# Parskatt/RoMa

Measured on AMD Instinct MI355X. Metric: image-pairs/sec, roma_outdoor 560->864, batch=8 per GPU, higher is better.
Workload: dtype bf16; 1 GPU; roma_outdoor match() 560->864, symmetric, upsample_preds, 8 pairs/GPU/step, seeded synthetic weights + N(0,1) images; precision policy of the reference's bf16 timing script: bfloat16 DINOv2 + float16 autocast for VGG / decoder / refiners (ROMA_MIXED), f32 accumulate; precision_policy=mixed, global_batch=8, streams_per_gpu=2, parallelism=single GPU, outputs_finite=True

## Files before the change

### include/roma_hip.h

```cpp
#ifndef ROMA_HIP_H
#define ROMA_HIP_H
#include <stdint.h>
#ifdef __cplusplus
extern "C" {
#endif

typedef struct roma_model* roma_handle_t;

enum { ROMA_F32 = 0, ROMA_BF16 = 1, ROMA_F16 = 2,
       ROMA_MIXED = 3 };
int roma_h16_format(void);
enum { ROMA_ERR_ARG = -1, ROMA_ERR_HIP = -2, ROMA_ERR_STATE = -3 };

typedef struct {
  int coarse_h, coarse_w;
  int upsample_h, upsample_w;
  int symmetric;
  int upsample_preds;
  int attenuate_cert;
  int precision;
  int max_batch;
  int device;
} roma_config_t;

// ... 52 lines not shown
int roma_debug_inject(roma_handle_t h, const char* name, const void* src_host, long nbytes);
long roma_debug_trace(roma_handle_t h, int slot, unsigned long long* sums_host, long max_entries, char* names_host,
                      long names_bytes);
int roma_destroy(roma_handle_t h);
int roma_tuning(const char* key, int value);
long roma_tuning_describe(char* buf, long nbytes);
long roma_debug_gemm_trace(unsigned int* dst_host, long nbytes);
int roma_profile_enable(int on);
long roma_profile_report(char* buf, long nbytes);


int roma_op_local_corr(const void* feature0, const void* feature1, const float* warp, void* out, int B, int H, int W,
                       int C, int K, int nearest, int dt_in, int dt_out, void* stream);
int roma_op_local_corr_window(const void* feature0, const void* feature1, const float* warp, void* out, int B, int H,
                              int W, int C, int radius, float scale, long ldo, int dt_in, int dt_out, void* stream);

int roma_op_gemm(const void* A, long lda, const void* W, long ldw, void* C, long ldc, int M, int N, int K, int batch,
                 long sA, long sW, long sC, const float* bias, const float* scale, const float* res, long ldr,
                 int act, float alpha, int dt_in, int dt_out, void* stream);
int roma_op_conv3x3(const void* in, const void* w, const float* bias, void* out, int B, int H, int W, int Cin, int Cout,
                    int relu, int dt, void* stream);
int roma_op_conv3x3_slab(const void* in, const void* w, const float* bias, void* out, int B, int H, int W, int Cin, int Cout,
                         int relu, int dt, void* stream);
int roma_op_attention(const void* q, const void* k, const void* vt, void* out, int B, int heads, int N, int npad, int hd,
                      int dt_in, int dt_out, void* stream);
int roma_op_qkv_scatter_gemm(const void* A, const void* W, const float* bias, void* q, void* k, void* vt, int B, int N,
                             int npad, int heads, int hd, int K, int dt_in, int dt_out, void* stream);
int roma_op_layernorm(const float* x, const float* w, const float* b, void* out, long M, int D, float eps, int dt_out,
                      void* stream);
int roma_op_layernorm_dt(const void* x, int dt_in, const float* w, const float* b, void* out, long M, int D, float eps,
// ... 107 lines not shown
```

### roma_amd/_lib.py

```python
from __future__ import annotations

import ctypes as C
import os

_HERE = os.path.dirname(os.path.abspath(__file__))
_HERE = os.environ.get("ROMA_LIB_DIR", _HERE)
LIB_PATH = os.path.join(_HERE, "libroma_hip.so")
LIB_PATHS = {"bf16": LIB_PATH, "f16": os.path.join(_HERE, "libroma_hip_f16.so")}

ROMA_F32, ROMA_BF16, ROMA_F16, ROMA_MIXED = 0, 1, 2, 3
H16_CODE = {"bf16": ROMA_BF16, "f16": ROMA_F16}


class RomaConfig(C.Structure):
    _fields_ = [("coarse_h", C.c_int), ("coarse_w", C.c_int), ("upsample_h", C.c_int), ("upsample_w", C.c_int),
                ("symmetric", C.c_int), ("upsample_preds", C.c_int), ("attenuate_cert", C.c_int),
                ("precision", C.c_int), ("max_batch", C.c_int), ("device", C.c_int)]


class RomaForwardArgs(C.Structure):
    _fields_ = [("upsample", C.c_int), ("symmetric", C.c_int), ("scale_factor", C.c_double),
                ("seed_flow", C.c_void_p), ("seed_cert", C.c_void_p), ("seed_h", C.c_int), ("seed_w", C.c_int),
                ("flow", C.c_void_p * 5), ("cert", C.c_void_p * 5), ("feat", C.c_void_p * 5)]

# ... 14 lines not shown
    "roma_match": (_i, [_vp, _i, _vp, _vp, _vp, _vp, _vp, _vp, _vp]),
    "roma_forward": (_i, [_vp, _i, _vp, _vp, C.POINTER(RomaForwardArgs), _vp]),
    "roma_debug_fetch": (_l, [_vp, C.c_char_p, _vp, _l]),
    "roma_debug_trace": (_l, [_vp, _i, _vp, _l, C.c_char_p, _l]),
    "roma_debug_inject": (_i, [_vp, C.c_char_p, _vp, _l]),
    "roma_destroy": (_i, [_vp]),
    "roma_tuning": (_i, [C.c_char_p, _i]),
    "roma_tuning_describe": (_l, [C.c_char_p, _l]),
    "roma_debug_gemm_trace": (_l, [_vp, _l]),
    "roma_vit_forward": (_i, [_vp, _vp]),
    "roma_op_convert_from_bf16": (_i, [_vp, _vp, _l, _vp]),
    "roma_profile_enable": (_i, [_i]),
    "roma_profile_report": (_l, [C.c_char_p, _l]),
    "roma_op_local_corr": (_i, [_vp, _vp, _vp, _vp, _i, _i, _i, _i, _i, _i, _i, _i, _vp]),
    "roma_op_local_corr_window": (_i, [_vp, _vp, _vp, _vp, _i, _i, _i, _i, _i, _f, _l, _i, _i, _vp]),
    "roma_op_gemm": (_i, [_vp, _l, _vp, _l, _vp, _l, _i, _i, _i, _i, _l, _l, _l, _vp, _vp, _vp, _l, _i, _f, _i, _i, _vp]),
    "roma_op_conv3x3": (_i, [_vp, _vp, _vp, _vp, _i, _i, _i, _i, _i, _i, _i, _vp]),
    "roma_op_conv3x3_slab": (_i, [_vp, _vp, _vp, _vp, _i, _i, _i, _i, _i, _i, _i, _vp]),
    "roma_op_attention": (_i, [_vp, _vp, _vp, _vp, _i, _i, _i, _i, _i, _i, _i, _vp]),
    "roma_op_qkv_scatter_gemm": (_i, [_vp, _vp, _vp, _vp, _vp, _vp, _i, _i, _i, _i, _i, _i, _i, _i, _vp]),
    "roma_op_layernorm": (_i, [_vp, _vp, _vp, _vp, _l, _i, _f, _i, _vp]),
    "roma_op_layernorm_dt": (_i, [_vp, _i, _vp, _vp, _vp, _l, _i, _f, _i, _vp]),
    "roma_op_gemm_res_bf16": (_i, [_vp, _l, _vp, _l, _vp, _l, _i, _i, _i, _vp, _vp, _vp, _l, _vp]),
    "roma_op_cholesky_solve_t": (_i, [_vp, _vp, _vp, _vp, _vp, _i, _i, _i, _vp]),
    "roma_op_gp": (_i, [_vp, _vp, _vp, _vp, _vp, _i, _i, _i, _i, _vp]),
    "roma_op_cls_to_flow": (_i, [_vp, _l, _vp, _vp, _l, _vp]),
    "roma_op_resize_bilinear": (_i, [_vp, _vp, _i, _i, _i, _i, _i, _i, _vp]),
    "roma_op_refiner_input": (_i, [_vp, _l, _vp, _vp, _l, _vp, _vp, _i, _i, _i, _i, _i, _i, _i, _i, _f, _i, _vp]),
    "roma_op_dwconv5x5": (_i, [_vp, _vp, _vp, _vp, _i, _i, _i, _i, _i, _vp]),
    "roma_op_refiner_block": (_i, [_vp, _vp, _vp, _vp, _vp, _vp, _i, _i, _i, _i, _i, _vp]),
# ... 86 lines not shown
```

### roma_amd/csrc/api.hip

```cpp
#include <algorithm>
#include <mutex>
#include <map>
#include <vector>
#include <dlfcn.h>
#include <string.h>

#include "../../include/roma_hip.h"
#include "attention.h"
#include "conv64.h"
#include "conv_patch.h"
#include "elementwise.h"
#include "gemm.h"
#include "local_corr.h"
#include "pool_proj.h"
#include "model.h"
#include "refiner_block.h"
#include "kde.h"
#include "keypoints.h"
#include "tiny.h"
#include "tuning.h"
#include "vit.h"
#include "sampling.h"
#include "sample_batched.h"
#include "essential.h"
// ... 286 lines not shown
  a.nearest = nearest ? 1 : 0;
  a.f0 = feature0; a.f1 = feature1; a.warp = warp; a.out = out; a.B = B; a.H = H; a.W = W; a.C = C; a.K = K;
  a.ld0 = C; a.ld1 = C; a.ldo = K; a.nimg = B; a.f1_shift = 0; a.scale = 1.f; a.in_dt = DT(dt_in); a.out_dt = DT(dt_out);
  return local_corr_general_launch(a, S(stream));
}

int roma_op_local_corr_window(const void* feature0, const void* feature1, const float* warp, void* out, int B, int H,
                              int W, int C, int radius, float scale, long ldo, int dt_in, int dt_out, void* stream) {
  LocalCorrArgs a;
  a.f0 = feature0; a.f1 = feature1; a.warp = warp; a.out = out; a.B = B; a.H = H; a.W = W; a.C = C; a.radius = radius;
  a.ld0 = C; a.ld1 = C; a.ldo = ldo; a.nimg = B; a.f1_shift = 0; a.scale = scale; a.in_dt = DT(dt_in); a.out_dt = DT(dt_out);
  ROMA_REQUIRE(ldo >= (2 * radius + 1) * (2 * radius + 1), "local_corr_window: ldo < K");
  return local_corr_window_launch(a, S(stream));
}

int roma_op_gemm(const void* A, long lda, const void* W, long ldw, void* C, long ldc, int M, int N, int K, int batch,
                 long sA, long sW, long sC, const float* bias, const float* scale, const float* res, long ldr, int act,
                 float alpha, int dt_in, int dt_out, void* stream) {
  GemmArgs g;
  g.A = A; g.lda = lda; g.W = W; g.ldw = ldw; g.C = C; g.ldc = ldc; g.M = M; g.N = N; g.K = K; g.batch = batch;
  g.sA = sA; g.sW = sW; g.sC = sC; g.bias = bias; g.scale = scale; g.res = res; g.ldr = ldr; g.sR = sC; g.act = act;
  g.alpha = alpha; g.in_dt = DT(dt_in); g.out_dt = DT(dt_out);
  return gemm_launch(g, S(stream));
}

int roma_op_conv3x3(const void* in, const void* w, const float* bias, void* out, int B, int H, int W, int Cin, int Cout,
                    int relu, int dt, void* stream) {
  GemmArgs g;
  g.A = in; g.W = w; g.ldw = 9 * Cin; g.C = out; g.ldc = Cout; g.M = B * H * W; g.N = Cout; g.K = 9 * Cin;
  g.in_dt = DT(dt); g.out_dt = DT(dt); g.bias = bias; g.act = relu ? ACT_RELU : ACT_NONE;
// ... 306 lines not shown
```

### roma_amd/csrc/chol_col.hip

```cpp
#include "chol_diag.h"
#include "elementwise.h"
#include "tuning.h"

namespace roma {

namespace {

struct CFrag { f32x4 v[8]; };

__device__ __forceinline__ void cc_load(CFrag& f, const float* p) {
#pragma unroll
  for (int q = 0; q < 8; ++q) f.v[q] = *reinterpret_cast<const f32x4*>(p + 4 * q);
}
__device__ __forceinline__ f32x16 cc_mfma(const CFrag& a, const CFrag& b, f32x16 acc) {
#pragma unroll
  for (int q = 0; q < 8; ++q)
#pragma unroll
    for (int u = 0; u < 4; ++u) acc = __builtin_amdgcn_mfma_f32_32x32x2f32(a.v[q][u], b.v[q][u], acc, 0, 0, 0);
  return acc;
}
__device__ __forceinline__ f32x16 cc_tile_product(const float* pa, const float* pb, int k) {
  f32x16 acc;
#pragma unroll
  for (int r = 0; r < 16; ++r) acc[r] = 0.f;
  CFrag a0, b0, a1, b1;
  if (k > 0) {
    cc_load(a0, pa);
    cc_load(b0, pb);
  }
  for (int t = 0; t < k; t += 2) {
    if (t + 1 < k) {
      cc_load(a1, pa + 64 * (t + 1));
      cc_load(b1, pb + 64 * (t + 1));
    }
    acc = cc_mfma(a0, b0, acc);
    if (t + 1 < k) {
      if (t + 2 < k) {
        cc_load(a0, pa + 64 * (t + 2));
        cc_load(b0, pb + 64 * (t + 2));
      }
      acc = cc_mfma(a1, b1, acc);
    }
  }
  return acc;
}

constexpr int CC_POLLS = 2000;

}

__global__ __launch_bounds__(256, 2) void chol_col_kernel(float* __restrict__ A, long ld, long strideA, float* __restrict__ LTm,
                                                          long strideLT, int n, float* __restrict__ Linv,
                                                          float* __restrict__ LinvT, int k, int nblk, unsigned epoch,
                                                          int use_leader) {
  constexpr int S = CHOL_S;
  __shared__ __attribute__((aligned(16))) float L[64 * S];
  __shared__ __attribute__((aligned(16))) float LT[64 * S];
  __shared__ __attribute__((aligned(16))) float XT[64 * S];
  __shared__ __attribute__((aligned(16))) float Pb[64 * S];
  __shared__ int progress;
  __shared__ int leader_ok;
  const int tid = threadIdx.x;
  const int wave = __builtin_amdgcn_readfirstlane(tid >> 6);
  const int lane = tid & 63, l31 = lane & 31, kk = lane >> 5;
  const int img = blockIdx.y;
  const bool split = use_leader && k > 0;
  const bool leader = split && blockIdx.x == 0;
  const int rb = split ? (int)blockIdx.x - 1 : (int)blockIdx.x;
  float* Ai = A + (long)img * strideA;
  const long S0 = 64l * k, R0 = 64l * (k + 1) + 64l * rb;
  unsigned* flag = reinterpret_cast<unsigned*>(LTm + (long)img * strideLT + n);
  const unsigned want = (epoch << 8) | (unsigned)(k + 1);
  float* Li = Linv + ((long)img * nblk + k) * 4096;
  float* LiT = LinvT + ((long)img * nblk + k) * 4096;
  if (tid == 0) {
    progress = -1;
    leader_ok = 0;
  }
  const int ti = wave >> 1, tj = wave & 1;

  if (!leader) {
    const float* pa = Ai + (R0 + 32 * ti + l31) * ld + 32 * kk;
    const float* pb = Ai + (S0 + 32 * tj + l31) * ld + 32 * kk;
    const f32x16 acc = cc_tile_product(pa, pb, k);
#pragma unroll
    for (int r = 0; r < 16; ++r) {
      const int row = 32 * ti + (r & 3) + 8 * (r >> 2) + 4 * kk, col = 32 * tj + l31;
      Pb[row * S + col] = Ai[(R0 + row) * ld + S0 + col] - acc[r];
    }
  }
  bool have_inverse = false;
  if (split && !leader) {
    if (tid == 0) {
      int ok = 0;
      for (int it = 0; it < CC_POLLS; ++it) {
        if (__hip_atomic_load(flag, __ATOMIC_RELAXED, __HIP_MEMORY_SCOPE_AGENT) == want) {
          ok = 1;
          break;
        }
// ... 2 lines not shown
      if (ok) __builtin_amdgcn_fence(__ATOMIC_ACQUIRE, "agent");
      leader_ok = ok;
    }
    __syncthreads();
    have_inverse = leader_ok != 0;
    if (have_inverse) {
      for (int idx = tid; idx < 64 * 16; idx += 256) {
        const int row = idx >> 4, c4 = (idx & 15) * 4;
        *reinterpret_cast<f32x4*>(&XT[row * S + c4]) = *reinterpret_cast<const f32x4*>(LiT + row * 64 + c4);
      }
    }
  }
  if (!have_inverse) {
    const float* pa = Ai + (S0 + 32 * ti + l31) * ld + 32 * kk;
    const float* pb = Ai + (S0 + 32 * tj + l31) * ld + 32 * kk;
    const f32x16 acc = cc_tile_product(pa, pb, k);
#pragma unroll
    for (int r = 0; r < 16; ++r) {
      const int row = 32 * ti + (r & 3) + 8 * (r >> 2) + 4 * kk, col = 32 * tj + l31;
      L[row * S + col] = Ai[(S0 + row) * ld + S0 + col] - acc[r];
    }
    __syncthreads();
    if (wave == 0) chol_diag_factor_wave(L, LT, &progress, lane);
    else if (wave == 1) chol_diag_inverse_wave(L, XT, &progress, lane);
  }
  __syncthreads();

  if (leader || (!split && rb == 0)) {
    chol_diag_writeback(L, XT, nullptr, ld, Li, LiT, tid, 256);
    float* ltd = LTm + (long)img * strideLT + S0 * (long)n + S0;
    for (int idx = tid; idx < 64 * 16; idx += 256) {
// ... 42 lines not shown
__global__ __launch_bounds__(256) void chol_col_restore_kernel(float* __restrict__ A, long ld, long strideA,
                                                               const float* __restrict__ LTm, long strideLT, int n) {
  __shared__ float tile[64 * 65];
  const int k = blockIdx.x, img = blockIdx.y, tid = threadIdx.x;
  const float* src = LTm + (long)img * strideLT + (64l * k) * n + 64l * k;
  float* dst = A + (long)img * strideA + (64l * k) * ld + 64l * k;
  for (int idx = tid; idx < 64 * 64; idx += 256) {
    const int r = idx >> 6, c = idx & 63;
    tile[r * 65 + c] = c >= r ? src[(long)r * n + c] : 0.f;
  }
  __syncthreads();
  for (int idx = tid; idx < 64 * 64; idx += 256) dst[(long)(idx >> 6) * ld + (idx & 63)] = tile[(idx & 63) * 65 + (idx >> 6)];
}

int chol_col_launch(float* A, long ld, long strideA, float* LT, long strideLT, int n, int d, float* Linv, float* LinvT, int k,
                    int nblk, int batch, unsigned epoch, hipStream_t s) {
  ROMA_REQUIRE(n % 64 == 0 && d % 64 == 0 && d >= 64 && ld % 4 == 0 && LT, "chol_col: n, d multiples of 64, d >= 64, ld of 4, LT");
  const int nrb = (n + d) / 64 - (k + 1);
  ROMA_REQUIRE(nrb >= 1 && k < nblk, "chol_col: no row block below the column");
  const int use_leader = tuning(SW_GP_COL_LEADER);
  const int gx = nrb + ((use_leader && k > 0) ? 1 : 0);
  hipLaunchKernelGGL(chol_col_kernel, dim3((unsigned)gx, (unsigned)batch), dim3(256), 0, s, A, ld, strideA, LT, strideLT, n, Linv,
                     LinvT, k, nblk, epoch & 0xffffffu, use_leader);
  ROMA_LAUNCH_CHECK();
  return 0;
}

int chol_col_restore_launch(float* A, long ld, long strideA, const float* LT, long strideLT, int n, int batch, hipStream_t s) {
  hipLaunchKernelGGL(chol_col_restore_kernel, dim3((unsigned)(n / 64), (unsigned)batch), dim3(256), 0, s, A, ld, strideA, LT,
                     strideLT, n);
  ROMA_LAUNCH_CHECK();
  return 0;
}

}
```

### roma_amd/csrc/elementwise.h

```cpp
#pragma once
#include "common.h"

namespace roma {

int layernorm_launch(const float* x, const float* w, const float* b, void* out, long M, int D, float eps,
                     int dt_out, hipStream_t s);
int layernorm_launch_dt(const void* x, int dt_in, const float* w, const float* b, void* out, long M, int D, float eps,
                        int dt_out, hipStream_t s);

int conv3x3_c3_launch(const float* img, const float* w, const float* bias, void* out, int B, int H, int W,
                      int dt_out, hipStream_t s);

int im2col3x3_c3_launch(const float* img, void* out, int B, int H, int W, int dt_out, hipStream_t s);

int maxpool2x2_launch(const void* in, void* out, int B, int H, int W, int C, int dt, hipStream_t s);

int im2col_patch14_launch(const float* img, void* out, int B, int H, int W, int Kpad, int dt_out, hipStream_t s);

int assemble_tokens_launch(const float* patch, const float* cls, const float* pos, float* tokens, int B, int T,
                           int D, hipStream_t s);

int copy2d_launch(const void* in, long ldi, int dt_in, void* out, long ldo, int dt_out, long rows, int cols,
                  hipStream_t s);

int convert_from_bf16_launch(const void* in, void* out, long n, hipStream_t s);

int rownorm_launch(const void* in, long ld, int dt, float* norms, long M, int C, hipStream_t s);

int gp_basis_launch(const float* w, const float* b, float* Ft, int Dg, int h, int wdt, int npad, hipStream_t s, int copies = 1,
                    long stride = 0);

int transpose_launch(const float* in, float* out, int n, long ld, int batch, hipStream_t s, long stride_in = 0, long stride_out = 0);

int chol_diag_launch(float* A, long ld, long strideA, float* Linv, float* LinvT, int k, int nblk, int batch,
                     hipStream_t s);

int chol_col_launch(float* A, long ld, long strideA, float* LT, long strideLT, int n, int d, float* Linv, float* LinvT, int k,
                    int nblk, int batch, unsigned epoch, hipStream_t s);
int chol_col_restore_launch(float* A, long ld, long strideA, const float* LT, long strideLT, int n, int batch, hipStream_t s);

int pad_identity_launch(float* A, long ld, long strideA, int n, int npad, int batch, hipStream_t s);

int cls_to_flow_launch(const float* logits, long ld, float* flow, float* cert, long M, hipStream_t s);

struct RefinerInputArgs {
  const void* feat = nullptr;
  long ldf = 0;
  const float* flow = nullptr;
  void* d = nullptr;
  long ldd = 0;
  const float* emb_w = nullptr;
  const float* emb_b = nullptr;
  int B = 0, H = 0, W = 0, C = 0, E = 0, Kcorr = 0, nimg = 0, shift = 0;
// ... 32 lines not shown
```

### roma_amd/csrc/local_corr.h

```cpp
#pragma once
#include "common.h"

namespace roma {

struct LocalCorrArgs {
  const void* f0 = nullptr;
  const void* f1 = nullptr;
  const float* warp = nullptr;
  void* out = nullptr;
  int B = 0, H = 0, W = 0, C = 0;
  int radius = 0;
  int K = 0;
  long ld0 = 0, ld1 = 0, ldo = 0;
  int nimg = 0, f1_shift = 0;
  float scale = 1.f;
  int in_dt = 0, out_dt = 0;
  int nearest = 0;
  int* ws = nullptr;
  long ws_bytes = 0;
  int force_gather = 0;
  int pxmax = 0;
  int bin_ts = 0, bin_nx = 0, bin_ny = 0, ws_bins = 0, ws_qlist = 0;
};

long local_corr_ws_ints(int B, int H, int W, int radius);

int local_corr_window_launch(const LocalCorrArgs& a, hipStream_t stream);
int local_corr_general_launch(const LocalCorrArgs& a, hipStream_t stream);

}
```

### roma_amd/csrc/local_corr.hip

```cpp
#include "local_corr.h"
#include "tuning.h"
#include <stdio.h>
#include <stdlib.h>
#include <algorithm>
#include "gemm.h"

namespace roma {

template <typename T> struct LcIO;
template <> struct LcIO<float> {
  static constexpr int CE = 4;
  __device__ static inline void ld(const float* p, float* v) {
    f32x4 x = *reinterpret_cast<const f32x4*>(p);
    v[0] = x[0]; v[1] = x[1]; v[2] = x[2]; v[3] = x[3];
  }
};
template <> struct LcIO<bf16_t> {
  static constexpr int CE = 8;
  __device__ static inline void ld(const bf16_t* p, float* v) {
    uint4 u = *reinterpret_cast<const uint4*>(p);
    v[0] = h16_lo(u.x); v[1] = h16_hi(u.x);
    v[2] = h16_lo(u.y); v[3] = h16_hi(u.y);
    v[4] = h16_lo(u.z); v[5] = h16_hi(u.z);
    v[6] = h16_lo(u.w); v[7] = h16_hi(u.w);
// ... 445 lines not shown
    const long bh = max(min(yhi + R + 1, a.H - 1) - max(ylo - R, 0) + 1, 0);
    coherent = bw * bh <= a.pxmax && !a.force_gather;
  }
  const unsigned long long mc = __ballot(valid && coherent), mg = __ballot(valid && !coherent);
  int basec = 0, baseg = 0;
  if (lane == 0) {
    if (mc) basec = atomicAdd(a.ws + 1, __popcll(mc));
    if (mg) baseg = atomicAdd(a.ws + 0, __popcll(mg));
  }
  basec = __shfl(basec, 0);
  baseg = __shfl(baseg, 0);
  const unsigned long long below = (1ull << lane) - 1ull;
  if (valid) {
    if (coherent) a.ws[4 + tiles + basec + __popcll(mc & below)] = tile;
    else a.ws[4 + baseg + __popcll(mg & below)] = tile;
  }
}

template <int R> __device__ __forceinline__ int lc_bin_of(const LocalCorrArgs& a, long pix, int b) {
  constexpr int P = 2 * R + 2;
  int x0, y0;
  float fx, fy;
  unnormalize_floor(a.warp[pix * 2 + 0], a.W, x0, fx);
  unnormalize_floor(a.warp[pix * 2 + 1], a.H, y0, fy);
  const int ox = min(max(x0 - R, -P), a.W), oy = min(max(y0 - R, -P), a.H);
  return (b * a.bin_ny + (oy + P) / a.bin_ts) * a.bin_nx + (ox + P) / a.bin_ts;
}

template <int R, bool SCATTER>
__global__ __launch_bounds__(64) void local_corr_bin_kernel(const LocalCorrArgs a) {
  const int li = blockIdx.x;
  const int nlist = a.ws[0];
  const int tile = a.ws[4 + li];
  if (li >= nlist) return;
  const int lane = threadIdx.x;
  const int tiles_x = (a.W + LC_TQ - 1) / LC_TQ, tiles_y = (a.H + LC_TQ - 1) / LC_TQ;
  const int tpi = tiles_x * tiles_y;
  const int b = tile / tpi;
  const int trem = tile - b * tpi;
  const int ty = trem / tiles_x, tx = trem - ty * tiles_x;
  const int gy = ty * LC_TQ + (lane >> 3), gx = tx * LC_TQ + (lane & 7);
  if (gy >= a.H || gx >= a.W) return;
  const long pix = (long)b * a.H * a.W + (long)gy * a.W + gx;
  const int bin = lc_bin_of<R>(a, pix, b);
  const int nbins = a.B * a.bin_nx * a.bin_ny;
  int* cnt = a.ws + a.ws_bins;
  if constexpr (!SCATTER) {
    atomicAdd(cnt + bin, 1);
  } else {
    const int slot = atomicAdd(cnt + 2 * nbins + bin, 1);
    a.ws[a.ws_qlist + (long)cnt[nbins + bin] * 64 + slot] = (int)pix;
  }
}

__global__ __launch_bounds__(1024) void local_corr_bin_scan_kernel(const LocalCorrArgs a) {
  __shared__ int part[1024];
  const int nbins = a.B * a.bin_nx * a.bin_ny;
  int* cnt = a.ws + a.ws_bins;
  const int tid = threadIdx.x;
  const int per = (nbins + 1023) / 1024;
  const int i0 = tid * per, i1 = min(i0 + per, nbins);
  int sum = 0;
  for (int i = i0; i < i1; ++i) sum += (cnt[i] + 63) >> 6;
  part[tid] = sum;
  __syncthreads();
  for (int off = 1; off < 1024; off <<= 1) {
    const int v = tid >= off ? part[tid - off] : 0;
    __syncthreads();
    part[tid] += v;
    __syncthreads();
  }
  int run = part[tid] - sum;
  for (int i = i0; i < i1; ++i) {
    cnt[nbins + i] = run;
    run += (cnt[i] + 63) >> 6;
  }
  if (tid == 1023) a.ws[2] = part[1023];
}

template <int R, typename T, typename TOUT, int NW>
__global__ __launch_bounds__(64 * NW) void local_corr_list_kernel(const LocalCorrArgs a) {
  extern __shared__ __attribute__((aligned(16))) float f0s[];
  constexpr int RPT = 64 / NW;
  const int li = blockIdx.x / RPT, rnd = blockIdx.x % RPT;
  const int nlist = a.ws[0];
  const int tile = a.ws[4 + li];
  if (li >= nlist) return;
  const int lane = threadIdx.x & 63, wave = threadIdx.x >> 6;
  const int tiles_x = (a.W + LC_TQ - 1) / LC_TQ, tiles_y = (a.H + LC_TQ - 1) / LC_TQ;
  const int tpi = tiles_x * tiles_y;
// ... 66 lines not shown
  ROMA_REQUIRE(a.nimg > 0, "local_corr: nimg must be positive");
  return 0;
}

static int lc_bin_ts(int radius) {
  const int P = 2 * radius + 2, pxmax = radius <= 3 ? 320 : 704;
  int ts = 1;
  while ((ts + P) * (ts + P) <= pxmax) ++ts;
  return ts;
}
long local_corr_ws_ints(int B, int H, int W, int radius) {
  if (radius != 2 && radius != 3 && radius != 7) return 0;
  const long tiles = (long)B * ((H + LC_TQ - 1) / LC_TQ) * ((W + LC_TQ - 1) / LC_TQ);
  const int ts = lc_bin_ts(radius), P = 2 * radius + 2;
  const long nbins = (long)B * ((W + P) / ts + 1) * ((H + P) / ts + 1);
  return 4 + 2 * tiles + 3 * nbins + 64 * (tiles + nbins);
}

template <int R, typename T, typename TOUT, bool MFMA>
static int launch_tiled(const LocalCorrArgs& a0, hipStream_t stream) {
  LocalCorrArgs a = a0;
  const int tiles = a.B * ((a.H + LC_TQ - 1) / LC_TQ) * ((a.W + LC_TQ - 1) / LC_TQ);
  constexpr int P = 2 * R + 2;
  a.bin_ts = lc_bin_ts(R);
  a.bin_nx = (a.W + P) / a.bin_ts + 1;
  a.bin_ny = (a.H + P) / a.bin_ts + 1;
  const long nbins = (long)a.B * a.bin_nx * a.bin_ny;
  a.ws_bins = 4 + 2 * tiles;
  a.ws_qlist = a.ws_bins + 3 * (int)nbins;
  const bool binned = tuning(SW_LC_BIN) != 0 && (long)a.B * a.H * a.W < (1l << 31) &&
                      (a.bin_ts + P - 1) * (a.bin_ts + P - 1) <= LcGeom<R, MFMA>::PXMAX;
  const size_t need = (size_t)local_corr_ws_ints(a.B, a.H, a.W, R) * sizeof(int);
  bool own_ws = false;
  if (!a.ws) {
    ROMA_CHECK_HIP(hipMallocAsync(reinterpret_cast<void**>(&a.ws), need, stream));
    own_ws = true;
  } else {
    ROMA_REQUIRE((size_t)a.ws_bytes >= need, "local_corr(window): work-list scratch too small");
  }
  a.force_gather = tuning_override(SW_LC_MODE) == 1 ? 1 : 0;
  ROMA_CHECK_HIP(hipMemsetAsync(a.ws, 0, 4 * sizeof(int), stream));
  const size_t lds_tile = (size_t)LcGeom<R, MFMA>::STAGE + 5 * 64 * 4 + 32;
  a.pxmax = LcGeom<R, MFMA>::PXMAX;
  static bool attr_set[64] = {false};
  int dev = 0;
  ROMA_CHECK_HIP(hipGetDevice(&dev));
  if (dev < 0 || dev >= 64 || !attr_set[dev]) {
    ROMA_CHECK_HIP(hipFuncSetAttribute(reinterpret_cast<const void*>(&local_corr_tile_kernel<R, T, TOUT, MFMA>),
                                       hipFuncAttributeMaxDynamicSharedMemorySize, (int)lds_tile));
    if (dev >= 0 && dev < 64) attr_set[dev] = true;
  }
  hipLaunchKernelGGL((local_corr_classify_kernel<R>), dim3((unsigned)((tiles + 63) / 64)), dim3(64), 0, stream, a);
  ROMA_LAUNCH_CHECK();
  hipLaunchKernelGGL((local_corr_tile_kernel<R, T, TOUT, MFMA>), dim3((unsigned)tiles), dim3(LcGeom<R, MFMA>::NTHR), lds_tile, stream, a);
  ROMA_LAUNCH_CHECK();
  if (binned) {
    ROMA_CHECK_HIP(hipMemsetAsync(a.ws + a.ws_bins, 0, (size_t)3 * nbins * sizeof(int), stream));
    ROMA_CHECK_HIP(hipMemsetAsync(a.ws + a.ws_qlist, 0xff, (size_t)64 * (tiles + nbins) * sizeof(int), stream));
    hipLaunchKernelGGL((local_corr_bin_kernel<R, false>), dim3((unsigned)tiles), dim3(64), 0, stream, a);
    ROMA_LAUNCH_CHECK();
    hipLaunchKernelGGL(local_corr_bin_scan_kernel, dim3(1), dim3(1024), 0, stream, a);
    ROMA_LAUNCH_CHECK();
    hipLaunchKernelGGL((local_corr_bin_kernel<R, true>), dim3((unsigned)tiles), dim3(64), 0, stream, a);
    ROMA_LAUNCH_CHECK();
    static bool attr_set_l[64] = {false};
    if (dev < 0 || dev >= 64 || !attr_set_l[dev]) {
      ROMA_CHECK_HIP(hipFuncSetAttribute(reinterpret_cast<const void*>(&local_corr_tile_kernel<R, T, TOUT, MFMA, true>),
                                         hipFuncAttributeMaxDynamicSharedMemorySize, (int)lds_tile));
      if (dev >= 0 && dev < 64) attr_set_l[dev] = true;
    }
    const long max_items = (long)tiles + nbins;
    hipLaunchKernelGGL((local_corr_tile_kernel<R, T, TOUT, MFMA, true>), dim3((unsigned)std::min<long>(max_items, 8192)), dim3(LcGeom<R, MFMA>::NTHR),
                       lds_tile, stream, a);
    ROMA_LAUNCH_CHECK();
  } else {
    hipLaunchKernelGGL((local_corr_list_kernel<R, T, TOUT, 4>), dim3((unsigned)tiles * 16u), dim3(256), (size_t)4 * a.C * sizeof(float),
                       stream, a);
    ROMA_LAUNCH_CHECK();
  }
// ... 70 lines not shown
```

### roma_amd/csrc/model.hip

```cpp
#include "model.h"

#include <dlfcn.h>
#include <math.h>
#include <stdlib.h>
#include <string.h>

#include <algorithm>
#include <atomic>
#include <set>

#include "attention.h"
#include "conv64.h"
#include "pool_proj.h"
#include "elementwise.h"
#include "gemm.h"
#include "local_corr.h"
#include "refiner_block.h"
#include "vit.h"

namespace roma {

std::mutex g_peer_mutex;
extern void* g_peer_lib;
extern int g_mixed_handles;
// ... 620 lines not shown
  return rc;
}

int cholesky_solve_t(float* A, float* Rt, float* LT, float* Linv, float* LinvT, int n, int d, int batch, hipStream_t st,
                     long strideA, long strideR) {
  ROMA_REQUIRE(n % 64 == 0 && n > 0 && d % 4 == 0, "cholesky_solve: n must be a multiple of 64, d of 4");
  const int nblk = n / 64;
  const long sA = strideA > 0 ? strideA : (long)n * n, sR = strideR > 0 ? strideR : (long)d * n, sL = (long)nblk * 4096;
  const long sLT = (long)n * n;
  const bool aug_env = tuning(SW_GP_AUG) != 0;
  const bool aug = aug_env && Rt == A + (long)n * n && (batch == 1 || (sA == sR && sA >= (long)(n + d) * n));
  const int extra = aug ? d : 0;
  const bool col = aug && tuning(SW_GP_COL) != 0 && d >= 64 && d % 64 == 0;
  static std::atomic<unsigned> solve_epoch{0};
  const unsigned epoch = col ? ++solve_epoch : 0u;
  for (int k = 0; k < nblk && col; ++k)
    if (int rc = chol_col_launch(A, n, sA, LT, sLT, n, d, Linv, LinvT, k, nblk, batch, epoch, st)) return rc;
  if (col)
    if (int rc = chol_col_restore_launch(A, n, sA, LT, sLT, n, batch, st)) return rc;
  for (int k = 0; k < nblk && !col; ++k) {
    if (int rc = chol_diag_launch(A, n, sA, Linv, LinvT, k, nblk, batch, st)) return rc;
    const int mrem = n - (k + 1) * 64;
    if (mrem + extra <= 0) break;
    GemmArgs g;
    g.A = A + (long)(k + 1) * 64 * n + k * 64; g.lda = n; g.sA = sA;
    g.W = Linv + (long)k * 4096; g.ldw = 64; g.sW = sL;
    g.C = const_cast<float*>(static_cast<const float*>(g.A)); g.ldc = n; g.sC = sA;
    g.M = mrem + extra; g.N = 64; g.K = 64; g.batch = batch;
    if (int rc = gemm_launch(g, st)) return rc;
    if (mrem <= 0) break;
    GemmArgs t;
    t.A = g.A; t.lda = n; t.sA = sA;
// ... 582 lines not shown
```

### roma_amd/csrc/tuning.hip

```cpp
#include "tuning.h"

#include <stdlib.h>
#include <string.h>

#include "../../include/roma_hip.h"

namespace roma {
void set_error(const std::string& msg);
namespace {

struct Row {
  Switch id;
  const char* key;
  const char* env;
  long def;
  int floor;
  bool tools_env;
  const char* doc;
};

constexpr Row ROWS[] = {
    {SW_GEMM8P, "gemm8p", "ROMA_GEMM8P", 1, 0, false, "large bf16 GEMMs on the 8-phase 256 x 256 kernel (1) or on the one-barrier-per-slab kernel (0)"},
    {SW_GEMM_DBG, "gemm_dbg", "ROMA_GEMM_DBG", 0, 0, false, "experiment bits of the GEMM kernels (1 skip output stores, 2 skip the K loop, 2048 no streaming stores, ...)"},
    {SW_GEMM8P_WALK, "gemm8p_walk", nullptr, -1, 1, false, "gemm8p: tile rows per group of the persistent walk (1 = row major); unset = 8 from 24 tile columns on, else 1"},
    {SW_GEMM8P_SCHED, "gemm8p_sched", "ROMA_GEMM8P_SCHED", 1, 0, false, "gemm8p K-loop schedule: 1 k-half phases, 0 quadrant phases (tools builds only)"},
    {SW_GEMM8P_MAXWG, "gemm8p_maxwg", nullptr, -1, 8, false, "gemm8p, measurement only: cap the persistent grid at n workgroups (a multiple of 8); unset = one per CU"},
    {SW_WS1X1, "ws1x1", "ROMA_WS1X1", 1, 0, false, "N = K = 576 refiner 1x1 on the weight-stationary kernel (1) or on the 256 x 192 tile kernel (0)"},
    {SW_LC_MODE, "lc_mode", "ROMA_LC_MODE", 0, 0, false, "local correlation: 0 tiled form + gather work list, 1 every tile on the gather list (key only), 2 per-pixel kernel"},
    {SW_LC_BIN, "lc_bin", "ROMA_LC_BIN", 1, 0, false, "local correlation: queries of incoherent tiles sorted by target bin (1) or gathered per query (0)"},
    {SW_CONV64, "conv64", "ROMA_CONV64", 7, 0, false, "weight-stationary VGG front end, bit mask: 1 the Cin = 64 kernels, 2 the Cin = 128 kernel, 4 the fused first layer"},
    {SW_CONV_PATCH, "conv_patch", "ROMA_CONV_PATCH", 1, 0, false, "patch-resident 3x3 kernel for slab-major VGG layers (1) or gemm8p (0); environment 0 also packs tap-major weights"},
    {SW_ATTN_XCD, "attn_xcd", "ROMA_ATTN_XCD", 1, 0, false, "attention work items in per-XCD bands of (batch, head) (1) or in plain order (0)"},
    {SW_ATTN_EXP2, "attn_exp2", nullptr, -1, 0, false, "tools only: force the 2^x softmax of the 16-bit attention kernel on / off; unset = as the caller says"},
    {SW_RB24W, "rb24w", "ROMA_RB24W", 1, 0, false, "C = 24 fused refiner block: wave-private kernel (1) or two-barrier workgroup kernel (0); consulted in tools builds only"},
    {SW_RB144_1B, "rb144_1b", "ROMA_RB144_1B", 1, 0, true, "C = 144 fused refiner block: one barrier per row (1) or two (0, tools builds only)"},
    {SW_RB_WIDE, "rb_wide", "ROMA_RB_WIDE", 0, 0, false, "C = 576 refiner block as one fused kernel (1; key 2 / 3 = with the scalar / packed stencil) or dwconv5x5 + 1x1 GEMM (0)"},
    {SW_DW_RING, "dw_ring", "ROMA_DW_RING", 1, 0, false, "depthwise 5x5: 0 register-prefetch kernel, 1 ring kernel for the large launches, 2 ring kernel for every shape it takes"},
    {SW_GP_COL, "gp_col", "ROMA_GP_COL", 1, 0, false, "GP Cholesky left-looking, one launch per block column (1) or the right-looking launch chain (0)"},
    {SW_POOL_PROJ, "pool_proj", "ROMA_POOL_PROJ", 1, 0, false, "max-pool + proj head of strides 1 / 2 in one pass (1) or as separate kernels (0)"},
    {SW_GP_COL_LEADER, "gp_col_leader", "ROMA_GP_COL_LEADER", 1, 0, false, "block-column Cholesky: one leader workgroup factorises the diagonal block (1) or every workgroup its own copy (0)"},
    {SW_GEMM8P_MINM, nullptr, "ROMA_GEMM8P_MINM", 2048, 0, false, "gemm8p: smallest M it takes for the wide (N >= 2048) dense launches"},
    {SW_GEMM_NT, nullptr, "ROMA_GEMM_NT", 1, 0, false, "non-temporal output stores in the 16-bit GEMM row writer"},
    {SW_GEMM_F32_FILL, nullptr, "ROMA_GEMM_F32_FILL", 1, 0, false, "exact-f32 GEMMs below 192 tiles of 256 x 256 run on 128 x 128 tiles"},
    {SW_GEMM_SMALLM, nullptr, "ROMA_GEMM_SMALLM", 1, 0, false, "GEMMs below 320 tiles of 128 x 128 run on 128 x 64 tiles"},
    {SW_CONV64_SY, nullptr, "ROMA_CONV64_SY", 0, 0, false, "conv64 strip height in rows; 0 = the split of H with the fewest rounds"},
    {SW_CONV_KORDER, nullptr, "ROMA_CONV_KORDER", 1, 0, false, "VGG layers with Cout >= 256 pack slab-major weight rows (read when a handle is created)"},
    {SW_RB_SY, nullptr, "ROMA_RB_SY", 0, 0, false, "fused refiner block strip height in rows; 0 = the split of H with the fewest rounds"},
    {SW_RB_DBG, nullptr, "ROMA_RB_DBG", 0, 0, true, "ablation bits of the two-barrier refiner block kernel"},
    {SW_RB_WIDE_PK, nullptr, "ROMA_RB_WIDE_PK", 1, 0, false, "rb_wide: packed (1) or scalar (0) stencil"},
    {SW_RBW_DBG, nullptr, "ROMA_RBW_DBG", 0, 0, true, "ablation bits of the rb_wide kernel (they produce wrong outputs by design)"},
    {SW_DWR_MAXSY, nullptr, "ROMA_DWR_MAXSY", 1 << 20, 0, false, "depthwise ring kernel: cap of the strip height in rows (at least 6)"},
    {SW_DW_RING_MINELEMS, nullptr, "ROMA_DW_RING_MINELEMS", 64l << 20, 0, false, "dw_ring = 1: smallest launch, in elements, that goes to the ring kernel"},
    {SW_RI_VEC, nullptr, "ROMA_RI_VEC", 1, 0, false, "refiner_input on the 16-byte vector kernel where alignment allows"},
    {SW_OUT_ROW, nullptr, "ROMA_OUT_ROW", 1, 0, false, "refiner_out: row kernel for C = 24 in 16-bit storage"},
    {SW_OUT_LPR, nullptr, "ROMA_OUT_LPR", 1, 0, false, "refiner_out, 16-bit: lanes per row chosen to fill the 16-byte pieces best"},
// ... 86 lines not shown
```

Baseline: 108.7 image-pairs/s.

## Sort local-corr queries with LDS counters and add Cholesky diagonal lookahead

The incoherent-tile binning in local correlation now runs as a banded sort kernel that counts and places queries with LDS atomics. This replaces the two workspace memsets and the per-tile device-atomic bin kernels, and a new entry point lets callers pass their own workspace. Separately, the block-column Cholesky kernel gets an extra workgroup that forms the next diagonal block's product one launch ahead and parks it, so the leader only adds the last k-slice. Both add workspace and grid complexity and change the order of floating-point accumulation.

```diff
diff --git a/include/roma_hip.h b/include/roma_hip.h
--- a/include/roma_hip.h
+++ b/include/roma_hip.h
@@ -90,6 +90,10 @@
                        int C, int K, int nearest, int dt_in, int dt_out, void* stream);
 int roma_op_local_corr_window(const void* feature0, const void* feature1, const float* warp, void* out, int B, int H,
                               int W, int C, int radius, float scale, long ldo, int dt_in, int dt_out, void* stream);
+long roma_op_local_corr_window_workspace(int B, int H, int W, int radius);
+int roma_op_local_corr_window_ws(const void* feature0, const void* feature1, const float* warp, void* out, int B, int H,
+                                 int W, int C, int radius, float scale, long ldo, int dt_in, int dt_out, void* ws,
+                                 long ws_bytes, void* stream);
 
 int roma_op_gemm(const void* A, long lda, const void* W, long ldw, void* C, long ldc, int M, int N, int K, int batch,
                  long sA, long sW, long sC, const float* bias, const float* scale, const float* res, long ldr,
diff --git a/roma_amd/_lib.py b/roma_amd/_lib.py
--- a/roma_amd/_lib.py
+++ b/roma_amd/_lib.py
@@ -52,6 +52,8 @@
     "roma_profile_report": (_l, [C.c_char_p, _l]),
     "roma_op_local_corr": (_i, [_vp, _vp, _vp, _vp, _i, _i, _i, _i, _i, _i, _i, _i, _vp]),
     "roma_op_local_corr_window": (_i, [_vp, _vp, _vp, _vp, _i, _i, _i, _i, _i, _f, _l, _i, _i, _vp]),
+    "roma_op_local_corr_window_workspace": (_l, [_i, _i, _i, _i]),
+    "roma_op_local_corr_window_ws": (_i, [_vp, _vp, _vp, _vp, _i, _i, _i, _i, _i, _f, _l, _i, _i, _vp, _l, _vp]),
     "roma_op_gemm": (_i, [_vp, _l, _vp, _l, _vp, _l, _i, _i, _i, _i, _l, _l, _l, _vp, _vp, _vp, _l, _i, _f, _i, _i, _vp]),
     "roma_op_conv3x3": (_i, [_vp, _vp, _vp, _vp, _i, _i, _i, _i, _i, _i, _i, _vp]),
     "roma_op_conv3x3_slab": (_i, [_vp, _vp, _vp, _vp, _i, _i, _i, _i, _i, _i, _i, _vp]),
diff --git a/roma_amd/csrc/api.hip b/roma_amd/csrc/api.hip
--- a/roma_amd/csrc/api.hip
+++ b/roma_amd/csrc/api.hip
@@ -324,6 +324,27 @@
   return local_corr_window_launch(a, S(stream));
 }
 
+long roma_op_local_corr_window_workspace(int B, int H, int W, int radius) {
+  if (B <= 0 || H <= 0 || W <= 0) return 0;
+  return local_corr_ws_ints(B, H, W, radius) * (long)sizeof(int);
+}
+
+int roma_op_local_corr_window_ws(const void* feature0, const void* feature1, const float* warp, void* out, int B, int H,
+                                 int W, int C, int radius, float scale, long ldo, int dt_in, int dt_out, void* ws,
+                                 long ws_bytes, void* stream) {
+  LocalCorrArgs a;
+  a.f0 = feature0; a.f1 = feature1; a.warp = warp; a.out = out; a.B = B; a.H = H; a.W = W; a.C = C; a.radius = radius;
+  a.ld0 = C; a.ld1 = C; a.ldo = ldo; a.nimg = B; a.f1_shift = 0; a.scale = scale; a.in_dt = DT(dt_in); a.out_dt = DT(dt_out);
+  a.ws = static_cast<int*>(ws); a.ws_bytes = ws_bytes;
+  ROMA_REQUIRE(ldo >= (2 * radius + 1) * (2 * radius + 1), "local_corr_window: ldo < K");
+  if (roma_op_local_corr_window_workspace(B, H, W, radius) == 0) {
+    a.ws = nullptr; a.ws_bytes = 0;
+  } else {
+    ROMA_REQUIRE(ws && (reinterpret_cast<uintptr_t>(ws) & 3) == 0, "local_corr_window_ws: ws must be a 4-byte aligned device pointer");
+  }
+  return local_corr_window_launch(a, S(stream));
+}
+
 int roma_op_gemm(const void* A, long lda, const void* W, long ldw, void* C, long ldc, int M, int N, int K, int batch,
                  long sA, long sW, long sC, const float* bias, const float* scale, const float* res, long ldr, int act,
                  float alpha, int dt_in, int dt_out, void* stream) {
diff --git a/roma_amd/csrc/chol_col.hip b/roma_amd/csrc/chol_col.hip
--- a/roma_amd/csrc/chol_col.hip
+++ b/roma_amd/csrc/chol_col.hip
@@ -1,6 +1,5 @@
 #include "chol_diag.h"
 #include "elementwise.h"
-#include "tuning.h"
 
 namespace roma {
 
@@ -19,23 +18,20 @@
     for (int u = 0; u < 4; ++u) acc = __builtin_amdgcn_mfma_f32_32x32x2f32(a.v[q][u], b.v[q][u], acc, 0, 0, 0);
   return acc;
 }
-__device__ __forceinline__ f32x16 cc_tile_product(const float* pa, const float* pb, int k) {
-  f32x16 acc;
-#pragma unroll
-  for (int r = 0; r < 16; ++r) acc[r] = 0.f;
+__device__ __forceinline__ f32x16 cc_tile_product(const float* pa, const float* pb, int t0, int t1, f32x16 acc) {
   CFrag a0, b0, a1, b1;
-  if (k > 0) {
-    cc_load(a0, pa);
-    cc_load(b0, pb);
-  }
-  for (int t = 0; t < k; t += 2) {
-    if (t + 1 < k) {
+  if (t0 < t1) {
+    cc_load(a0, pa + 64 * t0);
+    cc_load(b0, pb + 64 * t0);
+  }
+  for (int t = t0; t < t1; t += 2) {
+    if (t + 1 < t1) {
       cc_load(a1, pa + 64 * (t + 1));
       cc_load(b1, pb + 64 * (t + 1));
     }
     acc = cc_mfma(a0, b0, acc);
-    if (t + 1 < k) {
-      if (t + 2 < k) {
+    if (t + 1 < t1) {
+      if (t + 2 < t1) {
         cc_load(a0, pa + 64 * (t + 2));
         cc_load(b0, pb + 64 * (t + 2));
       }
@@ -44,6 +40,15 @@
   }
   return acc;
 }
+__device__ __forceinline__ f32x16 cc_zero() {
+  f32x16 acc;
+#pragma unroll
+  for (int r = 0; r < 16; ++r) acc[r] = 0.f;
+  return acc;
+}
+
+constexpr int CC_LA_PARK = 1;
+constexpr int CC_LA_CONSUME = 2;
 
 constexpr int CC_POLLS = 2000;
 
@@ -52,7 +57,7 @@
 __global__ __launch_bounds__(256, 2) void chol_col_kernel(float* __restrict__ A, long ld, long strideA, float* __restrict__ LTm,
                                                           long strideLT, int n, float* __restrict__ Linv,
                                                           float* __restrict__ LinvT, int k, int nblk, unsigned epoch,
-                                                          int use_leader) {
+                                                          int use_leader, int lookahead) {
   constexpr int S = CHOL_S;
   __shared__ __attribute__((aligned(16))) float L[64 * S];
   __shared__ __attribute__((aligned(16))) float LT[64 * S];
@@ -79,10 +84,21 @@
   }
   const int ti = wave >> 1, tj = wave & 1;
 
+  if ((lookahead & CC_LA_PARK) && blockIdx.x == gridDim.x - 1) {
+    const long S1 = S0 + 64;
+    const float* pa = Ai + (S1 + 32 * ti + l31) * ld + 32 * kk;
+    const float* pb = Ai + (S1 + 32 * tj + l31) * ld + 32 * kk;
+    const f32x16 acc = cc_tile_product(pa, pb, 0, k, cc_zero());
+    float* park = Li + 4096 + wave * 1024 + lane;
+#pragma unroll
+    for (int r = 0; r < 16; ++r) park[64 * r] = acc[r];
+    return;
+  }
+
   if (!leader) {
     const float* pa = Ai + (R0 + 32 * ti + l31) * ld + 32 * kk;
     const float* pb = Ai + (S0 + 32 * tj + l31) * ld + 32 * kk;
-    const f32x16 acc = cc_tile_product(pa, pb, k);
+    const f32x16 acc = cc_tile_product(pa, pb, 0, k, cc_zero());
 #pragma unroll
     for (int r = 0; r < 16; ++r) {
       const int row = 32 * ti + (r & 3) + 8 * (r >> 2) + 4 * kk, col = 32 * tj + l31;
@@ -115,7 +131,15 @@
   if (!have_inverse) {
     const float* pa = Ai + (S0 + 32 * ti + l31) * ld + 32 * kk;
     const float* pb = Ai + (S0 + 32 * tj + l31) * ld + 32 * kk;
-    const f32x16 acc = cc_tile_product(pa, pb, k);
+    int t0 = 0;
+    f32x16 acc = cc_zero();
+    if (leader && (lookahead & CC_LA_CONSUME)) {
+      const float* park = Li + wave * 1024 + lane;
+#pragma unroll
+      for (int r = 0; r < 16; ++r) acc[r] = park[64 * r];
+      t0 = k - 1;
+    }
+    acc = cc_tile_product(pa, pb, t0, k, acc);
 #pragma unroll
     for (int r = 0; r < 16; ++r) {
       const int row = 32 * ti + (r & 3) + 8 * (r >> 2) + 4 * kk, col = 32 * tj + l31;
@@ -188,14 +212,14 @@
 }
 
 int chol_col_launch(float* A, long ld, long strideA, float* LT, long strideLT, int n, int d, float* Linv, float* LinvT, int k,
-                    int nblk, int batch, unsigned epoch, hipStream_t s) {
+                    int nblk, int batch, unsigned epoch, int use_leader, hipStream_t s) {
   ROMA_REQUIRE(n % 64 == 0 && d % 64 == 0 && d >= 64 && ld % 4 == 0 && LT, "chol_col: n, d multiples of 64, d >= 64, ld of 4, LT");
   const int nrb = (n + d) / 64 - (k + 1);
   ROMA_REQUIRE(nrb >= 1 && k < nblk, "chol_col: no row block below the column");
-  const int use_leader = tuning(SW_GP_COL_LEADER);
-  const int gx = nrb + ((use_leader && k > 0) ? 1 : 0);
+  const int lookahead = use_leader != 1 ? 0 : (k >= 2 ? CC_LA_CONSUME : 0) | (k >= 1 && k + 1 < nblk ? CC_LA_PARK : 0);
+  const int gx = nrb + ((use_leader && k > 0) ? 1 : 0) + ((lookahead & CC_LA_PARK) ? 1 : 0);
   hipLaunchKernelGGL(chol_col_kernel, dim3((unsigned)gx, (unsigned)batch), dim3(256), 0, s, A, ld, strideA, LT, strideLT, n, Linv,
-                     LinvT, k, nblk, epoch & 0xffffffu, use_leader);
+                     LinvT, k, nblk, epoch & 0xffffffu, use_leader, lookahead);
   ROMA_LAUNCH_CHECK();
   return 0;
 }
diff --git a/roma_amd/csrc/elementwise.h b/roma_amd/csrc/elementwise.h
--- a/roma_amd/csrc/elementwise.h
+++ b/roma_amd/csrc/elementwise.h
@@ -36,7 +36,7 @@
                      hipStream_t s);
 
 int chol_col_launch(float* A, long ld, long strideA, float* LT, long strideLT, int n, int d, float* Linv, float* LinvT, int k,
-                    int nblk, int batch, unsigned epoch, hipStream_t s);
+                    int nblk, int batch, unsigned epoch, int use_leader, hipStream_t s);
 int chol_col_restore_launch(float* A, long ld, long strideA, const float* LT, long strideLT, int n, int batch, hipStream_t s);
 
 int pad_identity_launch(float* A, long ld, long strideA, int n, int npad, int batch, hipStream_t s);
diff --git a/roma_amd/csrc/local_corr.h b/roma_amd/csrc/local_corr.h
--- a/roma_amd/csrc/local_corr.h
+++ b/roma_amd/csrc/local_corr.h
@@ -21,6 +21,8 @@
   int force_gather = 0;
   int pxmax = 0;
   int bin_ts = 0, bin_nx = 0, bin_ny = 0, ws_bins = 0, ws_qlist = 0;
+  int sort_bands = 0;
+  long ws_tclass = 0, ws_hist = 0;
 };
 
 long local_corr_ws_ints(int B, int H, int W, int radius);
diff --git a/roma_amd/csrc/local_corr.hip b/roma_amd/csrc/local_corr.hip
--- a/roma_amd/csrc/local_corr.hip
+++ b/roma_amd/csrc/local_corr.hip
@@ -483,17 +483,21 @@
   if (valid) {
     if (coherent) a.ws[4 + tiles + basec + __popcll(mc & below)] = tile;
     else a.ws[4 + baseg + __popcll(mg & below)] = tile;
-  }
-}
-
-template <int R> __device__ __forceinline__ int lc_bin_of(const LocalCorrArgs& a, long pix, int b) {
+    if (a.sort_bands) a.ws[a.ws_tclass + tile] = coherent ? 1 : 0;
+  }
+}
+
+template <int R> __device__ __forceinline__ int lc_bin_in_image(const LocalCorrArgs& a, float wx, float wy) {
   constexpr int P = 2 * R + 2;
   int x0, y0;
   float fx, fy;
-  unnormalize_floor(a.warp[pix * 2 + 0], a.W, x0, fx);
-  unnormalize_floor(a.warp[pix * 2 + 1], a.H, y0, fy);
+  unnormalize_floor(wx, a.W, x0, fx);
+  unnormalize_floor(wy, a.H, y0, fy);
   const int ox = min(max(x0 - R, -P), a.W), oy = min(max(y0 - R, -P), a.H);
-  return (b * a.bin_ny + (oy + P) / a.bin_ts) * a.bin_nx + (ox + P) / a.bin_ts;
+  return ((oy + P) / a.bin_ts) * a.bin_nx + (ox + P) / a.bin_ts;
+}
+template <int R> __device__ __forceinline__ int lc_bin_of(const LocalCorrArgs& a, long pix, int b) {
+  return b * a.bin_ny * a.bin_nx + lc_bin_in_image<R>(a, a.warp[pix * 2 + 0], a.warp[pix * 2 + 1]);
 }
 
 template <int R, bool SCATTER>
@@ -522,15 +526,101 @@
   }
 }
 
+constexpr int LC_SORT_MAXBINS = 1024;
+constexpr int LC_SORT_MAXBANDS = 16;
+constexpr int LC_SORT_NTHR = 1024;
+constexpr int LC_SORT_U = 4;
+static inline int lc_sort_bands(int B, int tiles_y) {
+  return std::max(1, std::min(std::min((128 + B - 1) / B, LC_SORT_MAXBANDS), (tiles_y + 1) / 2));
+}
+
+template <int R, bool PLACE>
+__global__ __launch_bounds__(LC_SORT_NTHR) void local_corr_sort_kernel(const LocalCorrArgs a) {
+  __shared__ int tbl[LC_SORT_MAXBINS];
+  if (a.ws[0] == 0) return;
+  const int tid = threadIdx.x, lane = tid & 63;
+  const int wave = __builtin_amdgcn_readfirstlane(tid >> 6);
+  constexpr int NW = LC_SORT_NTHR / 64;
+  const int g = blockIdx.x, G = gridDim.x, b = blockIdx.y;
+  const int tiles_x = (a.W + LC_TQ - 1) / LC_TQ, tiles_y = (a.H + LC_TQ - 1) / LC_TQ;
+  const int tpi = tiles_x * tiles_y;
+  const int nb = a.bin_nx * a.bin_ny, nbins = a.B * nb;
+  const long HW = (long)a.H * a.W;
+  int* hist = a.ws + a.ws_hist + (long)b * G * nb;
+  int* ql = a.ws + a.ws_qlist;
+  const int* cnt = a.ws + a.ws_bins + (long)b * nb;
+  for (int i = tid; i < nb; i += LC_SORT_NTHR) {
+    int start = 0;
+    if constexpr (PLACE) {
+      const int first = cnt[nbins + i];
+#pragma unroll
+      for (int q = 0; q < LC_SORT_MAXBANDS; ++q) start += q < g ? hist[q * nb + i] : 0;
+      start += first * 64;
+      if (g == 0) {
+        const int c = cnt[i];
+        for (int s = c; s < ((c + 63) & ~63); ++s) ql[(long)first * 64 + s] = -1;
+      }
+    }
+    tbl[i] = start;
+  }
+  __syncthreads();
+  const int* tclass = a.ws + a.ws_tclass + (long)b * tpi;
+  const float2* warp = reinterpret_cast<const float2*>(a.warp) + (long)b * HW;
+  const int t1 = ((g + 1) * tiles_y / G) * tiles_x;
+  for (int tb = (g * tiles_y / G) * tiles_x + wave; tb < t1; tb += NW * LC_SORT_U) {
+    int qp[LC_SORT_U];
+    float2 wv[LC_SORT_U];
+#pragma unroll
+    for (int u = 0; u < LC_SORT_U; ++u) {
+      const int t = tb + NW * u;
+      const bool incoherent = t < t1 && tclass[min(t, t1 - 1)] == 0;
+      const int ty = t / tiles_x, tx = t - ty * tiles_x;
+      const int gy = ty * LC_TQ + (lane >> 3), gx = tx * LC_TQ + (lane & 7);
+      qp[u] = (incoherent && gy < a.H && gx < a.W) ? gy * a.W + gx : -1;
+    }
+#pragma unroll
+    for (int u = 0; u < LC_SORT_U; ++u) wv[u] = warp[max(qp[u], 0)];
+#pragma unroll
+    for (int u = 0; u < LC_SORT_U; ++u) {
+      if (qp[u] >= 0) {
+        const int slot = atomicAdd(&tbl[lc_bin_in_image<R>(a, wv[u].x, wv[u].y)], 1);
+        if constexpr (PLACE) ql[slot] = (int)((long)b * HW + qp[u]);
+      }
+    }
+  }
+  if constexpr (!PLACE) {
+    __syncthreads();
+    for (int i = tid; i < nb; i += LC_SORT_NTHR) hist[g * nb + i] = tbl[i];
+  }
+}
+
 __global__ __launch_bounds__(1024) void local_corr_bin_scan_kernel(const LocalCorrArgs a) {
   __shared__ int part[1024];
-  const int nbins = a.B * a.bin_nx * a.bin_ny;
+  const int nb = a.bin_nx * a.bin_ny, nbins = a.B * nb;
+  const int G = a.sort_bands;
+  if (G > 0 && a.ws[0] == 0) return;
   int* cnt = a.ws + a.ws_bins;
   const int tid = threadIdx.x;
   const int per = (nbins + 1023) / 1024;
   const int i0 = tid * per, i1 = min(i0 + per, nbins);
   int sum = 0;
-  for (int i = i0; i < i1; ++i) sum += (cnt[i] + 63) >> 6;
+  if (G > 0) {
+    const auto band_sum = [&](int i) {
+      const int* h = a.ws + a.ws_hist + (long)(i / nb) * G * nb + i % nb;
+      int c = 0;
+#pragma unroll
+      for (int q = 0; q < LC_SORT_MAXBANDS; ++q) c += q < G ? h[(long)q * nb] : 0;
+      return c;
+    };
+    for (int i = i0; i < i1; i += 2) {
+      const int c0 = band_sum(i), c1 = i + 1 < i1 ? band_sum(i + 1) : 0;
+      cnt[i] = c0;
+      if (i + 1 < i1) cnt[i + 1] = c1;
+      sum += ((c0 + 63) >> 6) + ((c1 + 63) >> 6);
+    }
+  } else {
+    for (int i = i0; i < i1; ++i) sum += (cnt[i] + 63) >> 6;
+  }
   part[tid] = sum;
   __syncthreads();
   for (int off = 1; off < 1024; off <<= 1) {
@@ -540,9 +630,12 @@
     __syncthreads();
   }
   int run = part[tid] - sum;
-  for (int i = i0; i < i1; ++i) {
+  for (int i = i0; i < i1; i += 2) {
+    const int c0 = cnt[i], c1 = i + 1 < i1 ? cnt[i + 1] : 0;
     cnt[nbins + i] = run;
-    run += (cnt[i] + 63) >> 6;
+    run += (c0 + 63) >> 6;
+    if (i + 1 < i1) cnt[nbins + i + 1] = run;
+    run += (c1 + 63) >> 6;
   }
   if (tid == 1023) a.ws[2] = part[1023];
 }
@@ -639,7 +732,7 @@
   const long tiles = (long)B * ((H + LC_TQ - 1) / LC_TQ) * ((W + LC_TQ - 1) / LC_TQ);
   const int ts = lc_bin_ts(radius), P = 2 * radius + 2;
   const long nbins = (long)B * ((W + P) / ts + 1) * ((H + P) / ts + 1);
-  return 4 + 2 * tiles + 3 * nbins + 64 * (tiles + nbins);
+  return 4 + 2 * tiles + 3 * nbins + 64 * (tiles + nbins) + tiles + lc_sort_bands(B, (H + LC_TQ - 1) / LC_TQ) * nbins;
 }
 
 template <int R, typename T, typename TOUT, bool MFMA>
@@ -653,8 +746,13 @@
   const long nbins = (long)a.B * a.bin_nx * a.bin_ny;
   a.ws_bins = 4 + 2 * tiles;
   a.ws_qlist = a.ws_bins + 3 * (int)nbins;
-  const bool binned = tuning(SW_LC_BIN) != 0 && (long)a.B * a.H * a.W < (1l << 31) &&
+  const int lc_bin = tuning(SW_LC_BIN);
+  const bool binned = lc_bin != 0 && (long)a.B * a.H * a.W < (1l << 31) &&
                       (a.bin_ts + P - 1) * (a.bin_ts + P - 1) <= LcGeom<R, MFMA>::PXMAX;
+  const bool lds_sort = binned && lc_bin == 1 && a.bin_nx * a.bin_ny <= LC_SORT_MAXBINS && 64 * ((long)tiles + nbins) < (1l << 31);
+  a.ws_tclass = a.ws_qlist + 64 * ((long)tiles + nbins);
+  a.ws_hist = a.ws_tclass + tiles;
+  a.sort_bands = lds_sort ? lc_sort_bands(a.B, (a.H + LC_TQ - 1) / LC_TQ) : 0;
   const size_t need = (size_t)local_corr_ws_ints(a.B, a.H, a.W, R) * sizeof(int);
   bool own_ws = false;
   if (!a.ws) {
@@ -680,14 +778,24 @@
   hipLaunchKernelGGL((local_corr_tile_kernel<R, T, TOUT, MFMA>), dim3((unsigned)tiles), dim3(LcGeom<R, MFMA>::NTHR), lds_tile, stream, a);
   ROMA_LAUNCH_CHECK();
   if (binned) {
-    ROMA_CHECK_HIP(hipMemsetAsync(a.ws + a.ws_bins, 0, (size_t)3 * nbins * sizeof(int), stream));
-    ROMA_CHECK_HIP(hipMemsetAsync(a.ws + a.ws_qlist, 0xff, (size_t)64 * (tiles + nbins) * sizeof(int), stream));
-    hipLaunchKernelGGL((local_corr_bin_kernel<R, false>), dim3((unsigned)tiles), dim3(64), 0, stream, a);
-    ROMA_LAUNCH_CHECK();
-    hipLaunchKernelGGL(local_corr_bin_scan_kernel, dim3(1), dim3(1024), 0, stream, a);
-    ROMA_LAUNCH_CHECK();
-    hipLaunchKernelGGL((local_corr_bin_kernel<R, true>), dim3((unsigned)tiles), dim3(64), 0, stream, a);
-    ROMA_LAUNCH_CHECK();
+    if (lds_sort) {
+      const dim3 sgrid((unsigned)a.sort_bands, (unsigned)a.B);
+      hipLaunchKernelGGL((local_corr_sort_kernel<R, false>), sgrid, dim3(LC_SORT_NTHR), 0, stream, a);
+      ROMA_LAUNCH_CHECK();
+      hipLaunchKernelGGL(local_corr_bin_scan_kernel, dim3(1), dim3(1024), 0, stream, a);
+      ROMA_LAUNCH_CHECK();
+      hipLaunchKernelGGL((local_corr_sort_kernel<R, true>), sgrid, dim3(LC_SORT_NTHR), 0, stream, a);
+      ROMA_LAUNCH_CHECK();
+    } else {
+      ROMA_CHECK_HIP(hipMemsetAsync(a.ws + a.ws_bins, 0, (size_t)3 * nbins * sizeof(int), stream));
+      ROMA_CHECK_HIP(hipMemsetAsync(a.ws + a.ws_qlist, 0xff, (size_t)64 * (tiles + nbins) * sizeof(int), stream));
+      hipLaunchKernelGGL((local_corr_bin_kernel<R, false>), dim3((unsigned)tiles), dim3(64), 0, stream, a);
+      ROMA_LAUNCH_CHECK();
+      hipLaunchKernelGGL(local_corr_bin_scan_kernel, dim3(1), dim3(1024), 0, stream, a);
+      ROMA_LAUNCH_CHECK();
+      hipLaunchKernelGGL((local_corr_bin_kernel<R, true>), dim3((unsigned)tiles), dim3(64), 0, stream, a);
+      ROMA_LAUNCH_CHECK();
+    }
     static bool attr_set_l[64] = {false};
     if (dev < 0 || dev >= 64 || !attr_set_l[dev]) {
       ROMA_CHECK_HIP(hipFuncSetAttribute(reinterpret_cast<const void*>(&local_corr_tile_kernel<R, T, TOUT, MFMA, true>),
diff --git a/roma_amd/csrc/model.hip b/roma_amd/csrc/model.hip
--- a/roma_amd/csrc/model.hip
+++ b/roma_amd/csrc/model.hip
@@ -658,8 +658,9 @@
   const bool col = aug && tuning(SW_GP_COL) != 0 && d >= 64 && d % 64 == 0;
   static std::atomic<unsigned> solve_epoch{0};
   const unsigned epoch = col ? ++solve_epoch : 0u;
+  const int col_leader = col ? (int)tuning(SW_GP_COL_LEADER) : 0;
   for (int k = 0; k < nblk && col; ++k)
-    if (int rc = chol_col_launch(A, n, sA, LT, sLT, n, d, Linv, LinvT, k, nblk, batch, epoch, st)) return rc;
+    if (int rc = chol_col_launch(A, n, sA, LT, sLT, n, d, Linv, LinvT, k, nblk, batch, epoch, col_leader, st)) return rc;
   if (col)
     if (int rc = chol_col_restore_launch(A, n, sA, LT, sLT, n, batch, st)) return rc;
   for (int k = 0; k < nblk && !col; ++k) {
diff --git a/roma_amd/csrc/tuning.hip b/roma_amd/csrc/tuning.hip
--- a/roma_amd/csrc/tuning.hip
+++ b/roma_amd/csrc/tuning.hip
@@ -27,7 +27,7 @@
     {SW_GEMM8P_MAXWG, "gemm8p_maxwg", nullptr, -1, 8, false, "gemm8p, measurement only: cap the persistent grid at n workgroups (a multiple of 8); unset = one per CU"},
     {SW_WS1X1, "ws1x1", "ROMA_WS1X1", 1, 0, false, "N = K = 576 refiner 1x1 on the weight-stationary kernel (1) or on the 256 x 192 tile kernel (0)"},
     {SW_LC_MODE, "lc_mode", "ROMA_LC_MODE", 0, 0, false, "local correlation: 0 tiled form + gather work list, 1 every tile on the gather list (key only), 2 per-pixel kernel"},
-    {SW_LC_BIN, "lc_bin", "ROMA_LC_BIN", 1, 0, false, "local correlation: queries of incoherent tiles sorted by target bin (1) or gathered per query (0)"},
+    {SW_LC_BIN, "lc_bin", "ROMA_LC_BIN", 1, 0, false, "local correlation: queries of incoherent tiles sorted by target bin, counters in LDS (1) or device atomics (2), or gathered per query (0)"},
     {SW_CONV64, "conv64", "ROMA_CONV64", 7, 0, false, "weight-stationary VGG front end, bit mask: 1 the Cin = 64 kernels, 2 the Cin = 128 kernel, 4 the fused first layer"},
     {SW_CONV_PATCH, "conv_patch", "ROMA_CONV_PATCH", 1, 0, false, "patch-resident 3x3 kernel for slab-major VGG layers (1) or gemm8p (0); environment 0 also packs tap-major weights"},
     {SW_ATTN_XCD, "attn_xcd", "ROMA_ATTN_XCD", 1, 0, false, "attention work items in per-XCD bands of (batch, head) (1) or in plain order (0)"},
@@ -38,7 +38,7 @@
     {SW_DW_RING, "dw_ring", "ROMA_DW_RING", 1, 0, false, "depthwise 5x5: 0 register-prefetch kernel, 1 ring kernel for the large launches, 2 ring kernel for every shape it takes"},
     {SW_GP_COL, "gp_col", "ROMA_GP_COL", 1, 0, false, "GP Cholesky left-looking, one launch per block column (1) or the right-looking launch chain (0)"},
     {SW_POOL_PROJ, "pool_proj", "ROMA_POOL_PROJ", 1, 0, false, "max-pool + proj head of strides 1 / 2 in one pass (1) or as separate kernels (0)"},
-    {SW_GP_COL_LEADER, "gp_col_leader", "ROMA_GP_COL_LEADER", 1, 0, false, "block-column Cholesky: one leader workgroup factorises the diagonal block (1) or every workgroup its own copy (0)"},
+    {SW_GP_COL_LEADER, "gp_col_leader", "ROMA_GP_COL_LEADER", 1, 0, false, "block-column Cholesky: a leader workgroup factorises the diagonal block, its product formed one launch ahead (1) or in its own launch (2), or every workgroup its own copy (0)"},
     {SW_GEMM8P_MINM, nullptr, "ROMA_GEMM8P_MINM", 2048, 0, false, "gemm8p: smallest M it takes for the wide (N >= 2048) dense launches"},
     {SW_GEMM_NT, nullptr, "ROMA_GEMM_NT", 1, 0, false, "non-temporal output stores in the 16-bit GEMM row writer"},
     {SW_GEMM_F32_FILL, nullptr, "ROMA_GEMM_F32_FILL", 1, 0, false, "exact-f32 GEMMs below 192 tiles of 256 x 256 run on 128 x 128 tiles"},
```

New measurement: 110.4 image-pairs/s, median of 6. 1.02x the previous value.
